# pvphan/camera-calibration

Hardware: AMD Instinct MI355X
Metric: LM iters/sec & residuals/sec, 10k-view checkerboard @1/2/4/8 GPU (higher is better)
Workload: dtype f64

## Files before the change

### camera-calibration_amd/csrc/kernels.hpp

```cpp
#pragma once
#include "point_model.hpp"
#include <stdint.h>
#include <type_traits>

namespace calib {

constexpr int kTile = 256;
constexpr int kGramChunk = 512;
constexpr int kGramUnroll = 4;
constexpr int kGRows = 0;
constexpr int kGStride = 96;
__host__ __device__ __forceinline__ constexpr int gvSlot(int L, int j) { return j < 5 ? L + 1 + j : 16 + L + 2; }
__host__ __device__ __forceinline__ constexpr int gvOfSlot(int L, int slot) {
    const int m = slot >> 4, n = (slot & 15) - L;
    return (m == 0 && n >= 1 && n <= 5) ? n - 1 : ((m == 1 && n == 2) ? 5 : -1);
}
constexpr int kPartStride = 112;
constexpr int kMaxL = 10;

constexpr int kEmitZero = 256;
constexpr int kEmitTile = 264;
constexpr int kEmitTabSize = kGStride + kPartStride;
inline void buildEmitTable(int C, uint32_t* tab ) {
    const int L = C - 6;
// ... 19 lines not shown
        for (int c = 0; c < 16; ++c) tab[kGRows + m * 16 + c] = entry(L + m, c);
    for (int j = 0; j < 6; ++j) tab[gvSlot(L, j)] = gentry(L + j);
    uint32_t* part = tab + kGStride;
    for (int r = 0; r < L; ++r)
        for (int c = 0; c < L; ++c) part[r * L + c] = entry(r, c);
    for (int c = 0; c < L; ++c) part[L * L + c] = gentry(c);
    part[L * L + L] = sse;
}

__host__ __device__ __forceinline__ constexpr int64_t jIndex(int64_t p, int c, int C) {
    return ((p >> 2) * C + c) * 4 + (p & 3);
}
constexpr int kSchurThreads = 256;
constexpr int kMaxSchurBlocks = 1024;

typedef double d4 __attribute__((ext_vector_type(4)));
typedef float f4 __attribute__((ext_vector_type(4)));

__device__ __forceinline__ double2 lane_gather(double2 v, int srcLane) {
    const int a = srcLane << 2;
    int2 lo = __builtin_bit_cast(int2, v.x), hi = __builtin_bit_cast(int2, v.y);
    lo.x = __builtin_amdgcn_ds_bpermute(a, lo.x);  lo.y = __builtin_amdgcn_ds_bpermute(a, lo.y);
    hi.x = __builtin_amdgcn_ds_bpermute(a, hi.x);  hi.y = __builtin_amdgcn_ds_bpermute(a, hi.y);
    double2 o;
    o.x = __builtin_bit_cast(double, lo);  o.y = __builtin_bit_cast(double, hi);
    return o;
}
__device__ __forceinline__ float2 lane_gather(float2 v, int srcLane) {
    const int a = srcLane << 2;
    float2 o;
    o.x = __builtin_bit_cast(float, __builtin_amdgcn_ds_bpermute(a, __builtin_bit_cast(int, v.x)));
    o.y = __builtin_bit_cast(float, __builtin_amdgcn_ds_bpermute(a, __builtin_bit_cast(int, v.y)));
    return o;
}

struct LMState {
    double lam, err_cur, last_err, lam_min, lam_max, err_min;
    int cur;
    int round;
    int iters;
    int max_iters;
    int done;
    int error;
    int accepted_last;
    int fixed_mask;
    int* notify;
    double dc[kMaxL];
    double B[kMaxL * kMaxL];
    double gc[kMaxL];
};

__host__ __device__ constexpr int variantSize(int L) { return 2 * L * L + 2 * L + 2; }
__host__ __device__ constexpr int reduceSize(int L) { return 2 * variantSize(L); }

__device__ __forceinline__ const double* selectP(const double* P0, const double* P1,
                                                 const LMState* st, int sel) {
    if (sel == 0) return P0;
    return (st->cur ^ 1) ? P1 : P0;
}

template <typename T>
__global__ void view_setup_kernel(const double* __restrict__ P0, const double* __restrict__ P1,
                                  const LMState* __restrict__ st, int sel, int L,
                                  const int* __restrict__ view_ext, int nv, T* __restrict__ VC) {
    if (sel && st->done) return;
    const int j = blockIdx.x * blockDim.x + threadIdx.x;
// ... 160 lines not shown
        gacc += __shfl_xor(gacc, 16, 64);
        gacc += __shfl_xor(gacc, 32, 64);
        eacc += __shfl_xor(eacc, 16, 64);
        eacc += __shfl_xor(eacc, 32, 64);
    }
    double* Gbase = sel ? ((st->cur ^ 1) ? G1 : G0) : G0;
#pragma unroll
    for (int reg = 0; reg < 4; ++reg) stile[wave][(k + 4 * reg) * 16 + c] = acc[reg];
    if (k == 0) stile[wave][256 + c] = gacc;
    if (lane == 0) stile[wave][272] = eacc;
    __syncthreads();
    if (threadIdx.x < L * L + L + 1) {
        const int t = threadIdx.x;
        const int idx = t < L * L ? (t / L) * 16 + t % L : (t < L * L + L ? 256 + (t - L * L) : 272);
        part[(int64_t)(part_base + blockIdx.x) * kPartStride + t] =
            (stile[0][idx] + stile[1][idx]) + (stile[2][idx] + stile[3][idx]);
    }
    if (sub == 0 && valid) {
        double* G = Gbase + (int64_t)item * kGStride;
        for (int i = lane; i < kGStride; i += 64) {
            const int j = gvOfSlot(L, i);
            const int idx = j >= 0 ? 256 + L + j : (L + i / 16) * 16 + i % 16;
            double t = stile[wave][idx];
            for (int w = 1; w < wpi; ++w) t += stile[wave + w][idx];
            G[i] = t;
        }
    }
}

constexpr int kFusedRowChunks = 17;
constexpr int kFusedRows = 32;
constexpr int kFusedWaves = 4;

template <typename T, int C>
struct FusedSlab {
    using T2 = typename Pair<T>::type;
    static constexpr bool MF32 = sizeof(T) == 4;
    static constexpr int RS = kFusedRowChunks, ROWS = kFusedRows, WAVES = kFusedWaves;
    static constexpr bool RCOL = C < 16;
    static constexpr bool ONES = !RCOL;
    static constexpr int SIZE = MF32 ? ROWS * RS : ROWS * 16 + ROWS / 2;
    static constexpr int BYTES = WAVES * SIZE * (int)sizeof(T2);
    static_assert(SIZE * sizeof(T2) >= 2 * kEmitTile * 8, "tiles must fit the wave's slab");
    static __device__ __forceinline__ constexpr int rowOff(int r) { return MF32 ? r * RS : r * 16 + (r >> 1); }
    static __device__ __forceinline__ int pointOf(int lane) {
        return MF32 ? lane : ((lane & 48) | ((lane & 7) << 1) | ((lane >> 3) & 1));
    }
    static __device__ __forceinline__ void initRows(T2* slab, int lane) {
        if (lane < ROWS) {
            T2 c3, c4;
            c3.x = T(1); c3.y = ONES ? T(1) : T(0);
            c4.x = T(0); c4.y = T(1);
            slab[rowOff(lane) + 3] = c3;
            if (!ONES) slab[rowOff(lane) + 4] = c4;
            T* zr = reinterpret_cast<T*>(slab + rowOff(lane));
            zr[1] = T(0); zr[2] = T(0); zr[5] = T(0);
        }
    }
    static __device__ __forceinline__ double* tileU(T2* slab) { return reinterpret_cast<double*>(slab); }
    static __device__ __forceinline__ double* tileV(T2* slab) { return tileU(slab) + kEmitTile; }
    static __device__ __forceinline__ void writePartial(const unsigned char* smem, const uint32_t* emit_tab, double* part) {
        if ((int)threadIdx.x < kPartStride) {
            const uint32_t t = emit_tab[kGStride + threadIdx.x];
            const double* T0 = reinterpret_cast<const double*>(smem);
            double o = 0.0;
#pragma unroll
            for (int w = 0; w < WAVES; ++w) {
                const double* TUw = reinterpret_cast<const double*>(reinterpret_cast<const T2*>(T0) + w * SIZE);
                o += TUw[t & 0xffff] + (TUw + kEmitTile)[t >> 16];
            }
            part[(int64_t)blockIdx.x * kPartStride + threadIdx.x] = o;
        }
    }
};

struct BlockAcc {
    double d0u = 0.0, d0v = 0.0, d1u = 0.0, d1v = 0.0, d2u = 0.0;
    int bi, bj, trow, tcol0, tcol1, tcol2;
    __device__ __forceinline__ explicit BlockAcc(int lane) {
        const int k = lane >> 4;
        bi = (lane >> 2) & 3; bj = lane & 3;
        trow = 4 * bi + k; tcol0 = 4 * bi + bj; tcol1 = 4 * ((bi + 1) & 3) + bj; tcol2 = 4 * ((bi + 2) & 3) + bj;
    }
    __device__ __forceinline__ void contract(const double2& ja, const double2& jb, double ha, double hc) {
        d0u = __builtin_amdgcn_mfma_f64_4x4x4f64(ja.x, ja.x, d0u, 0, 0, 0);
        d0v = __builtin_amdgcn_mfma_f64_4x4x4f64(ja.y, ja.y, d0v, 0, 0, 0);
        d1u = __builtin_amdgcn_mfma_f64_4x4x4f64(ja.x, jb.x, d1u, 0, 0, 0);
        d1v = __builtin_amdgcn_mfma_f64_4x4x4f64(ja.y, jb.y, d1v, 0, 0, 0);
        d2u = __builtin_amdgcn_mfma_f64_4x4x4f64(ha, hc, d2u, 0, 0, 0);
    }
    __device__ __forceinline__ void park(double* TU, double* TV) const {
        TU[trow * 16 + tcol0] = d0u;  TV[trow * 16 + tcol0] = d0v;
        TU[trow * 16 + tcol1] = d1u;  TV[trow * 16 + tcol1] = d1v;
        TU[tcol1 * 16 + trow] = d1u;  TV[tcol1 * 16 + trow] = d1v;
        double* T2nd = bi < 2 ? TU : TV;
        T2nd[trow * 16 + tcol2] = d2u;
        T2nd[tcol2 * 16 + trow] = d2u;
    }
};

template <int MODEL, typename T, bool G44, bool MULTI>
__global__ __launch_bounds__(64 * kFusedWaves, (sizeof(T) == 4 ? (MULTI ? 5 : 6)
                                                             : (ModelTraits<MODEL>::C == 16 ? 4 : 3))) void fused_kernel(const double* __restrict__ P0, const double* __restrict__ P1,
                                                    const typename Pair<T>::type* __restrict__ uv,
                                                    const typename Pair<T>::type* __restrict__ XY,
                                                    const T* __restrict__ Z, const T* __restrict__ VC,
                                                    const int64_t* __restrict__ item_pt0,
                                                    const int* __restrict__ item_n,
                                                    const int* __restrict__ item_view, int n_items,
                                                    int uniform_n, int ipw, int wpi,
                                                    const uint32_t* __restrict__ emit_tab,
                                                    const LMState* __restrict__ st, int sel,
                                                    double* __restrict__ G0, double* __restrict__ G1,
                                                    double* __restrict__ part) {
    using T2 = typename Pair<T>::type;
    constexpr int C = ModelTraits<MODEL>::C;
    using Slab = FusedSlab<T, C>;
    constexpr int RS = Slab::RS, ROWS = Slab::ROWS, WAVES = Slab::WAVES, SLAB = Slab::SIZE;
    constexpr bool MF32 = Slab::MF32, RCOL = Slab::RCOL, ONES = Slab::ONES;
    __shared__ __attribute__((aligned(16))) unsigned char smem[Slab::BYTES];
    if (sel && st->done) return;
    const double* P = selectP(P0, P1, st, sel);
    const int lane = threadIdx.x & 63;
    const int wave = __builtin_amdgcn_readfirstlane(threadIdx.x >> 6);
    const int lw = wpi == 4 ? 2 : (wpi == 2 ? 1 : 0);
    const int sub = wave & (wpi - 1);
    static_assert(!(G44 && MULTI), "multi-item waves exist for the tile forms only");
    const int item_first = MULTI ? (blockIdx.x * WAVES + wave) * ipw : blockIdx.x * (WAVES >> lw) + (wave >> lw);
    const bool valid = item_first < n_items;
    int item = item_first;
    const int c = lane & 15, k = lane >> 4;
    const int sl = MF32 ? lane : ((lane & 48) | ((lane & 7) << 1) | ((lane >> 3) & 1));
    T2* slab = reinterpret_cast<T2*>(smem) + wave * SLAB;
    d4 acc = {0.0, 0.0, 0.0, 0.0}, acc2 = {0.0, 0.0, 0.0, 0.0};
    BlockAcc blk(lane);
    double* Gbase = sel ? ((st->cur ^ 1) ? G1 : G0) : G0;
    auto emitDirect = [&](int it) {
        constexpr int L = C - 6, RESROW = RCOL ? 15 : 4;
        double* G = Gbase + (int64_t)it * kGStride;
#pragma unroll
        for (int reg = 0; reg < 4; ++reg) {
            const int row = MF32 ? 4 * k + reg : k + 4 * reg;
            double val = acc[reg] + acc2[reg];
            if (ONES) {
                const int lo = __builtin_amdgcn_update_dpp(0, __double2loint(acc2[reg]), 0x111, 0xf, 0xf, false);
                const int hi = __builtin_amdgcn_update_dpp(0, __double2hiint(acc2[reg]), 0x111, 0xf, 0xf, false);
                const double fromLeft = __hiloint2double(hi, lo);
                val = c == 3 ? acc[reg] : (c == 4 ? fromLeft : val);
            }
            if (row >= L && row < L + 6) {
                const int slot = kGRows + (row - L) * 16 + c;
                if (gvOfSlot(L, slot) < 0) G[slot] = (RCOL && c == 15) ? 0.0 : val;
            } else if (row == RESROW) {
                if (c >= L && c < L + 6) G[gvSlot(L, c - L)] = val;
            }
        }
    };
    if (valid) {
        int64_t pbeg = uniform_n ? (int64_t)item * uniform_n : item_pt0[item];
        const int n = uniform_n ? uniform_n : item_n[item];
        const int item_last = MULTI ? (item_first + ipw < n_items ? item_first + ipw : n_items) - 1 : item_first;
        const int per = ((((n + 3) >> 2) + wpi - 1) >> lw) << 2;
        const int qbeg = sub * per;
        const int qend = qbeg + per < n ? qbeg + per : n;
        Shared<MODEL, T> sp;
        sp.load(P);
        Slab::initRows(slab, lane);
        int64_t pn = pbeg + (qbeg + sl < qend ? qbeg + sl : qend - 1);
        T2 m_n = uv[pn], xy_n = XY[pn];
        T z_n = Z[pn];
        for (;; ++item) {
        const T* vc = VC + (int64_t)__builtin_amdgcn_readfirstlane(uniform_n ? item : item_view[item]) * kViewStride;
        for (int q0 = qbeg; q0 < qend; q0 += 64) {
            const int q = q0 + sl;
            const T2 m = m_n, xy = xy_n;
            const T z = z_n;
            if (q0 + 64 < qend) {
                pn = pbeg + (q + 64 < qend ? q + 64 : qend - 1);
                m_n = uv[pn]; xy_n = XY[pn]; z_n = Z[pn];
            } else if (MULTI && item < item_last) {
                pn = pbeg + n + (sl < n ? sl : n - 1);
                m_n = uv[pn]; xy_n = XY[pn]; z_n = Z[pn];
            }
            T u, v;
            T2 Jc[C];
            jacobian_point<MODEL, T>(sp, vc, xy.x, xy.y, z, u, v, Jc);
            T2 res;
            res.x = m.x - u;
            res.y = m.y - v;
            constexpr int NCH = C - 5 + 1;
            T2 ch[NCH];
#pragma unroll
            for (int i = 0; i < C - 5; ++i) ch[i] = Jc[5 + i];
            ch[NCH - 1] = res;
            auto colOf = [](int i) { return i < C - 5 ? 5 + i : (RCOL ? 15 : 4); };
#pragma unroll
            for (int i = 0; i + 1 < NCH; i += 2) {
                unsigned a[sizeof(T2) / 4], b[sizeof(T2) / 4];
                __builtin_memcpy(a, &ch[i], sizeof(T2));
                __builtin_memcpy(b, &ch[i + 1], sizeof(T2));
#pragma unroll
                for (int d = 0; d < (int)(sizeof(T2) / 4); ++d) {
                    const auto r = __builtin_amdgcn_permlane32_swap(a[d], b[d], false, false);
// ... 64 lines not shown
                    const T* h2 = reinterpret_cast<const T*>(src + c2) + jh;
                    if (rows >= ROWS) {
#pragma unroll
                        for (int s = 0; s < ROWS / 4; ++s)
                            blk.contract(src[66 * s + c], src[66 * s + c1], h0[2 * 66 * s], h2[2 * 66 * s]);
                    } else {
                        for (int s = 0; s < nfull; ++s)
                            blk.contract(src[66 * s + c], src[66 * s + c1], h0[2 * 66 * s], h2[2 * 66 * s]);
                        if (rows & 3) {
                            const bool live = 4 * nfull + k < rows;
                            T2 ja = src[66 * nfull + c], jb = src[66 * nfull + c1];
                            double ha = h0[2 * 66 * nfull], hc = h2[2 * 66 * nfull];
                            if (!live) { ja.x = T(0); ja.y = T(0); jb.x = T(0); jb.y = T(0); ha = 0.0; hc = 0.0; }
                            blk.contract(ja, jb, ha, hc);
                        }
                    }
                }
            }
        }
        if (!MULTI || item >= item_last) break;
        emitDirect(item);
        {
            constexpr int L = C - 6;
#pragma unroll
            for (int reg = 0; reg < 4; ++reg) {
                const int row = MF32 ? 4 * k + reg : k + 4 * reg;
                const bool ofView = (row >= L && row < L + 6) || (c >= L && c < L + 6);
                acc[reg] = ofView ? 0.0 : acc[reg];
                acc2[reg] = ofView ? 0.0 : acc2[reg];
            }
        }
        pbeg += n;
        }
    }
    double* TU = Slab::tileU(slab);
    double* TV = Slab::tileV(slab);
    if (!G44 && wpi == 1 && valid) emitDirect(item);
    __builtin_amdgcn_wave_barrier();
    if constexpr (!G44) {
#pragma unroll
        for (int reg = 0; reg < 4; ++reg) {
            const int row = MF32 ? 4 * k + reg : k + 4 * reg;
            TU[row * 16 + c] = acc[reg];
            TV[row * 16 + c] = acc2[reg];
        }
    } else {
        blk.park(TU, TV);
    }
    if (lane == 0) { TU[kEmitZero] = 0.0; TV[kEmitZero] = 0.0; }
    __syncthreads();
    Slab::writePartial(smem, emit_tab, part);
    if ((!G44 && wpi == 1) || sub != 0 || !valid) return;
    double* G = Gbase + (int64_t)item * kGStride;
    if (lane < kGStride / 2) {
        const int i0 = 2 * lane;
        const uint2 t = *reinterpret_cast<const uint2*>(emit_tab + i0);
        double2 o;
        o.x = TU[t.x & 0xffff] + TV[t.x >> 16];
        o.y = TU[t.y & 0xffff] + TV[t.y >> 16];
        for (int w = 1; w < wpi; ++w) {
            const double* TUw = reinterpret_cast<const double*>(slab + w * SLAB);
            const double* TVw = TUw + kEmitTile;
            o.x += TUw[t.x & 0xffff] + TVw[t.x >> 16];
            o.y += TUw[t.y & 0xffff] + TVw[t.y >> 16];
        }
        *reinterpret_cast<double2*>(G + i0) = o;
    }
}

constexpr int kStreamOps = 12;
constexpr int kStreamNoOp = 0x7ffffff0;
inline bool buildStreamOps(int C, int32_t* ops ) {
    uint32_t tab[kEmitTabSize];
    buildEmitTable(C, tab);
    for (int i = 0; i < 64 * kStreamOps; ++i) ops[i] = kStreamNoOp;
    struct Src { int lane, acc; };
    const auto laneOf = [](int k, int b, int x) { return k * 16 + b * 4 + x; };
    const auto locate = [&](int idx, bool vtile) -> Src {
        const int r = idx / 16, c = idx % 16, br = r / 4, bc = c / 4;
        if (bc == br) return {laneOf(r % 4, br, c % 4), vtile ? 1 : 0};
        if (bc == ((br + 1) & 3)) return {laneOf(r % 4, br, c % 4), vtile ? 3 : 2};
        if (br == ((bc + 1) & 3)) return {laneOf(c % 4, bc, r % 4), vtile ? 3 : 2};
        const bool own = vtile ? br >= 2 : br < 2;
        return own ? Src{laneOf(r % 4, br, c % 4), 4} : Src{laneOf(c % 4, bc, r % 4), 4};
// ... 14 lines not shown
            else if (su.acc == 4 && sv.acc == 4) put(su.lane, 4, 2, slot);
            else ok = false;
        } else if (iu != kEmitZero) {
            const Src su = locate(iu, false);
            put(su.lane, su.acc == 0 ? 6 : (su.acc == 2 ? 8 : 10), 1, slot);
        } else {
            const Src sv = locate(iv, true);
            put(sv.lane, sv.acc == 1 ? 7 : (sv.acc == 3 ? 9 : 10), 1, slot);
        }
    }
    return ok;
}

constexpr int kStreamMinBlocks = 4;
template <int MODEL>
__global__ __launch_bounds__(64 * kFusedWaves, kStreamMinBlocks) void fused_stream_kernel(const double* __restrict__ P0, const double* __restrict__ P1,
                                                              const double2* __restrict__ uv, const double2* __restrict__ XY,
                                                              const double* __restrict__ Z, const double* __restrict__ VC,
                                                              int n, int nv, int share,
                                                              const uint32_t* __restrict__ emit_tab,
                                                              const int32_t* __restrict__ stream_ops,
                                                              const LMState* __restrict__ st, int sel,
                                                              double* __restrict__ G0, double* __restrict__ G1,
                                                              double* __restrict__ part) {
    using T = double;
    using T2 = double2;
    constexpr int C = ModelTraits<MODEL>::C, L = C - 6;
    using Slab = FusedSlab<T, C>;
    constexpr int ROWS = Slab::ROWS, WAVES = Slab::WAVES, SLAB = Slab::SIZE;
    constexpr bool RCOL = Slab::RCOL, ONES = Slab::ONES;
    __shared__ __attribute__((aligned(16))) unsigned char smem[Slab::BYTES];
    __shared__ __attribute__((aligned(16))) double svc[WAVES][2 * kViewStride];
    __shared__ __attribute__((aligned(16))) int32_t sops[64 * kStreamOps];
    int fin = 0, useP1 = 0;
    auto readState = [&]() {
        if (sel) {
            fin = st->done;
            useP1 = st->cur ^ 1;
        }
    };
    const int lane = threadIdx.x & 63;
    const int wave = __builtin_amdgcn_readfirstlane(threadIdx.x >> 6);
    const int k = lane >> 4;
    const int sl = Slab::pointOf(lane);
    T2* slab = reinterpret_cast<T2*>(smem) + wave * SLAB;
    BlockAcc blk(lane);
    double* Gbase = G0;
    auto ofView = [](int i) { return i >= L && i < L + 6; };
    const bool keep0 = !(ofView(blk.trow) || ofView(blk.tcol0)), keep1 = !(ofView(blk.trow) || ofView(blk.tcol1)),
               keep2 = !(ofView(blk.trow) || ofView(blk.tcol2));
    {
        const int4* src = reinterpret_cast<const int4*>(stream_ops) + 3 * lane;
        int4* dst = reinterpret_cast<int4*>(sops) + 3 * lane;
        dst[0] = src[0]; dst[1] = src[1]; dst[2] = src[2];
    }
    const int partner = blk.bj * 16 + ((blk.bi + 2) & 3) * 4 + k;
    auto emitView = [&](int slot) {
        typedef unsigned int u2v __attribute__((ext_vector_type(2)));
        const unsigned long long gp = reinterpret_cast<unsigned long long>(Gbase + (int64_t)slot * kGStride);
        const unsigned glo = (unsigned)__builtin_amdgcn_readfirstlane((int)(unsigned)gp);
        const unsigned ghi = (unsigned)__builtin_amdgcn_readfirstlane((int)(unsigned)(gp >> 32));
        double* G = reinterpret_cast<double*>(((unsigned long long)ghi << 32) | (unsigned long long)glo);
        const auto rsrc = __builtin_amdgcn_make_buffer_rsrc(G, 0, kGStride * 8, 0x00020000);
        const int4* o4 = reinterpret_cast<const int4*>(sops) + 3 * lane;
        const int4 oa = o4[0], ob = o4[1];
        double &d0u = blk.d0u, &d0v = blk.d0v, &d1u = blk.d1u, &d1v = blk.d1v, &d2u = blk.d2u;
        const double s0 = d0u + d0v, s1 = d1u + d1v;
        const double dp = __hiloint2double(__builtin_amdgcn_ds_bpermute(partner << 2, __double2hiint(d2u)),
                                           __builtin_amdgcn_ds_bpermute(partner << 2, __double2loint(d2u)));
        const double s2 = d2u + dp;
        auto put = [&](int off, double val) {
            __builtin_amdgcn_raw_buffer_store_b64(__builtin_bit_cast(u2v, val), rsrc, off, 0, 0);
        };
        put(oa.x, s0); put(oa.y, s0);
        put(oa.z, s1); put(oa.w, s1);
        put(ob.x, s2); put(ob.y, s2);
        if (ONES) {
            const int4 oc = o4[2];
            put(ob.z, d0u); put(ob.w, d0v);
            put(oc.x, d1u); put(oc.y, d1v);
            put(oc.z, d2u);
        }
        d0u = keep0 ? d0u : 0.0;  d0v = keep0 ? d0v : 0.0;
        d1u = keep1 ? d1u : 0.0;  d1v = keep1 ? d1v : 0.0;
        d2u = keep2 ? d2u : 0.0;
    };
    const int n4 = n >> 2;
    const int w = blockIdx.x * WAVES + wave;
    const long long gt = (long long)nv * n4, g0 = (long long)w * share;
    const bool valid = g0 < gt;
    if (valid) {
        const int p0 = (int)(4 * g0);
        const int p1 = (int)(4 * (g0 + share < gt ? g0 + share : gt));
        int va = __builtin_amdgcn_readfirstlane(p0 / n);
        int vend = (va + 1) * n;
        int slot = p0 != va * n ? nv + w : va;
        Shared<MODEL, T> sp, spB;
        sp.load(P0);
        spB = sp;
        if (sel) spB.load(P1);
        Slab::initRows(slab, lane);
        int pn = p0 + sl < p1 ? p0 + sl : p1 - 1;
        T2 m_n = uv[pn], xy_n = XY[pn];
        T z_n = Z[pn];
        auto straddles = [&](int q0, int ve) { return ve > q0 && ve < (q0 + 64 < p1 ? q0 + 64 : p1); };
        const int vcLast = nv * kViewStride - 1;
        auto stagedLoad = [&](int view) {
            const int i = view * kViewStride + (lane < 2 * kViewStride ? lane : 2 * kViewStride - 1);
            return VC[i < vcLast ? i : vcLast];
        };
        double vc_n = 0.0;
        double vcs[kViewStride];
#pragma unroll
        for (int i = 0; i < kViewStride; ++i) vcs[i] = 0.0;
        auto scalarLoad = [&](int view) {
            const T* s = VC + (int64_t)__builtin_amdgcn_readfirstlane(view) * kViewStride;
#pragma unroll
            for (int i = 0; i < kViewStride - 1; ++i) vcs[i] = s[i];
        };
        bool strad = straddles(p0, vend);
        if (strad) vc_n = stagedLoad(va); else scalarLoad(va);
        readState();
        if (fin) return;
        if (useP1) sp = spB;
        Gbase = useP1 ? G1 : G0;
        const T2* src = slab + Slab::rowOff(k);
        const int c = lane & 15, c1 = (c + 4) & 15, c2 = (c + 8) & 15, jh = (lane >> 3) & 1;
        const T* h0 = reinterpret_cast<const T*>(src + c) + jh;
        const T* h2 = reinterpret_cast<const T*>(src + c2) + jh;
        PointState<MODEL, T> pst;
        for (int q0 = p0; q0 < p1; q0 += 64) {
            const int qe = q0 + 64 < p1 ? q0 + 64 : p1;
            const int q = q0 + sl;
            const T2 m = m_n, xy = xy_n;
            const T z = z_n;
            const double vcx = vc_n;
            const bool more = q0 + 64 < p1;
            const bool passes = vend < qe;
            const int ve2 = passes ? vend + n : vend, va2 = passes ? va + 1 : va;
            const bool strad2 = more && straddles(q0 + 64, ve2);
            const int vfirst2 = ve2 <= q0 + 64 ? va2 + 1 : va2;
            if (more) {
                pn = q + 64 < p1 ? q + 64 : p1 - 1;
                m_n = uv[pn]; xy_n = XY[pn]; z_n = Z[pn];
                if (strad2) vc_n = stagedLoad(va2);
            }
            T u, v;
            T2 Jc[C];
            if (!strad) {
                jacobian_stage_a<MODEL, T>(sp, vcs, xy.x, xy.y, z, pst);
                jacobian_stage_b<MODEL, T>(sp, vcs, pst, u, v, Jc);
            } else {
                double* sv = svc[wave];
                if (lane < 2 * kViewStride) sv[lane] = vcx;
                __builtin_amdgcn_wave_barrier();
                const int qc = q < p1 ? q : p1 - 1;
                const double2* s2 = reinterpret_cast<const double2*>(sv + (qc >= vend ? kViewStride : 0));
                T vcl[kViewStride];
// ... 83 lines not shown
                        runFixed(integral_constant<int, 0>{}, integral_constant<int, JB>{});
                        nextView();
                        runFixed(integral_constant<int, JB>{}, integral_constant<int, NG>{});
                    };
                    switch (jb) {
                    case 0: boundaryAt(integral_constant<int, 0>{}); break;
                    case 1: boundaryAt(integral_constant<int, 1>{}); break;
                    case 2: boundaryAt(integral_constant<int, 2>{}); break;
                    case 3: boundaryAt(integral_constant<int, 3>{}); break;
                    case 4: boundaryAt(integral_constant<int, 4>{}); break;
                    case 5: boundaryAt(integral_constant<int, 5>{}); break;
                    case 6: boundaryAt(integral_constant<int, 6>{}); break;
                    default: boundaryAt(integral_constant<int, 7>{}); break;
                    }
                } else {
                    const int sb = jb < ng ? jb : ng;
                    auto runGroups = [&](int from, int to) {
                        switch (from) {
#define CALIB_GROUP_CASE(S) case S: if (to <= S) break; blk.contract(src[66 * S + c], src[66 * S + c1], h0[2 * 66 * S], h2[2 * 66 * S]); [[fallthrough]];
                        CALIB_GROUP_CASE(0) CALIB_GROUP_CASE(1) CALIB_GROUP_CASE(2) CALIB_GROUP_CASE(3)
                        CALIB_GROUP_CASE(4) CALIB_GROUP_CASE(5) CALIB_GROUP_CASE(6) CALIB_GROUP_CASE(7)
#undef CALIB_GROUP_CASE
                        default: break;
                        }
                    };
                    runGroups(0, sb);
                    if (jb < ng) {
                        nextView();
                        runGroups(sb, ng);
                    }
                }
            }
        }
        emitView(slot);
    } else {
        readState();
        if (fin) return;
    }
    {
        double* TU = Slab::tileU(slab);
        double* TV = Slab::tileV(slab);
        __builtin_amdgcn_wave_barrier();
        blk.park(TU, TV);
        if (lane == 0) { TU[kEmitZero] = 0.0; TV[kEmitZero] = 0.0; }
    }
    __syncthreads();
    Slab::writePartial(smem, emit_tab, part);
}

struct StreamMap { int share, n4, nv; };
__host__ __device__ __forceinline__ int stream_extra_item(const StreamMap& sm, int v) {
    if (sm.share == 0) return -1;
    const unsigned first = (unsigned)v * (unsigned)sm.n4, last = first + (unsigned)sm.n4 - 1u;
    const unsigned w = last / (unsigned)sm.share;
    return w * (unsigned)sm.share > first ? sm.nv + (int)w : -1;
}

struct ViewSpan { int i0, nitems, extra; };
template <bool STREAM>
__device__ __forceinline__ ViewSpan view_span(const int* __restrict__ view_item0, const StreamMap& sm, int v) {
    ViewSpan s;
    s.i0 = view_item0 ? view_item0[v] : v;
    s.nitems = view_item0 ? view_item0[v + 1] - s.i0 : 1;
    s.extra = STREAM ? stream_extra_item(sm, v) : -1;
    return s;
}

__device__ __forceinline__ constexpr int tri(int m, int n) { return m * (m + 1) / 2 + n; }

__device__ __forceinline__ double rsqrt_nr(double d) {
    const double r = __builtin_amdgcn_rsq(d);
    const double e = __builtin_fma(-(d * r), r, 1.0);
    const double p = __builtin_fma(0.375, e, 0.5);
    return __builtin_fma(r * e, p, r);
}

template <int N>
__device__ __forceinline__ double row_bcast(double v) {
    return __hiloint2double(__builtin_amdgcn_update_dpp(0, __double2hiint(v), 0x150 + N, 0xf, 0xf, false),
                            __builtin_amdgcn_update_dpp(0, __double2loint(v), 0x150 + N, 0xf, 0xf, false));
// ... 161 lines not shown
    __shared__ double sfail[kSchurViewsPerBlock];
    __shared__ double stile[kSchurBlock / 64][256];
    const int tid = threadIdx.x, lane = tid & 63, wave = tid >> 6, c = tid & 15, grp = tid >> 4, k = lane >> 4;

    if (blockIdx.y == 2) {
        constexpr int NF = L * L + L + 1;
        double* out = part + (int64_t)blockIdx.x * VA;
        const int t = tid & 127, half = tid >> 7;
        double s0 = 0.0, s1 = 0.0, s2 = 0.0, s3 = 0.0;
        if (t < NF) {
            const int64_t step = (int64_t)gridDim.x * 2;
            int64_t it = (int64_t)blockIdx.x * 2 + half;
            const double* src = bpart + t;
            for (; it + 3 * step < n_bpart; it += 4 * step) {
                s0 += src[it * kPartStride];
                s1 += src[(it + step) * kPartStride];
                s2 += src[(it + 2 * step) * kPartStride];
                s3 += src[(it + 3 * step) * kPartStride];
            }
            for (; it < n_bpart; it += step) s0 += src[it * kPartStride];
        }
        if (st->done) return;
        double* sh = &stile[0][0];
        sh[tid] = (s0 + s1) + (s2 + s3);
        __syncthreads();
        if (tid < NF) {
            const double tot = sh[tid] + sh[128 + tid];
            out[tid < L * L ? tid : (tid < L * L + L ? 2 * L * L + (tid - L * L) : kSse)] = tot;
        }
        return;
    }

    const double* G = blockIdx.y ? G1 : G0;
    double V[21], b[6];
    int v0 = blockIdx.x * kSchurViewsPerBlock;
    if (v0 + grp < nv) load_view_head<L, WIDE>(G, view_span<STREAM>(view_item0, sm, v0 + grp), c, V, b);
    if (st->done) return;
    const bool boot = st->round == 0;
    const int cand = st->cur ^ 1;
    const int variant = (int)blockIdx.y == cand ? 0 : 1;
    double* out = part + ((int64_t)variant * gridDim.x + blockIdx.x) * VA;
    if (variant == 1 && boot) {
        for (int i = tid; i < VA; i += kSchurBlock) out[i] = 0.0;
        return;
    }
    const double lam = variant == 0 ? (boot ? st->lam : st->lam / 10) : st->lam * 10;

    d4 acc = {0.0, 0.0, 0.0, 0.0};
    double nfail = 0.0;
    const int stride = gridDim.x * kSchurViewsPerBlock;
    while (v0 < nv) {
        double z[6];
#pragma unroll
        for (int m = 0; m < 6; ++m) z[m] = 0.0;
        const bool live = v0 + grp < nv;
        const bool more = v0 + stride + grp < nv;
        double rn[6];
        if (WIDE && more)
            request_head_rows(G, view_span<STREAM>(view_item0, sm, v0 + stride + grp), c, rn);
        if (live) {
            double invd[6];
            const bool ok = eliminate(V, b, lam, invd, z);
            if (c > L) {
#pragma unroll
                for (int m = 0; m < 6; ++m) z[m] = 0.0;
            }
            if (!ok) nfail += 1.0;
        }
        v0 += stride;
        if (more) {
            if constexpr (WIDE) {
                expand_head_rows<L>(rn, c, V, b);
            } else {
                load_view_head<L, false>(G, view_span<STREAM>(view_item0, sm, v0 + grp), c, V, b);
            }
        }
#pragma unroll
        for (int m = 0; m < 6; ++m) acc = __builtin_amdgcn_mfma_f64_16x16x4f64(z[m], z[m], acc, 0, 0, 0);
    }
// ... 68 lines not shown
        u32x4 mine;
        mine.x = (unsigned)__double2loint(t); mine.y = x.epoch;
        mine.z = (unsigned)__double2hiint(t); mine.w = x.epoch;
        if (lane != x.rank) cell_store(dst, mine);
        const unsigned long long* src = own + 2 * ((int64_t)(lane * 2 + par) * kPeerStride + i);
        const long long t0 = wall_clock64();
        v = t;
        while (lane != x.rank) {
            const u32x4 c = cell_load(src);
            if (c.y == x.epoch && c.w == x.epoch) {
                v = __hiloint2double((int)c.z, (int)c.x);
                break;
            }
            if ((unsigned long long)(wall_clock64() - t0) > x.timeout_ticks) {
                __hip_atomic_store(x.fault, 1, __ATOMIC_RELAXED, __HIP_MEMORY_SCOPE_AGENT);
                if (x.notify) __hip_atomic_store(x.notify, 2, __ATOMIC_RELAXED, __HIP_MEMORY_SCOPE_SYSTEM);
                v = __builtin_nan("");
                break;
            }
            __builtin_amdgcn_s_sleep(2);
        }
    }
    double acc = 0.0;
    for (int r = 0; r < x.world; ++r) acc += __shfl(v, r, 64);
    return acc;
}

__global__ __launch_bounds__(64) void reduce_kernel(const double* __restrict__ part, int nblocks, int VA,
                                                    const LMState* __restrict__ st,
                                                    double* __restrict__ red, PeerExchange x) {
    const int i = blockIdx.x, lane = threadIdx.x;
    const int variant = i / VA, idx = i - variant * VA;
    const double* src = part + (int64_t)variant * nblocks * VA + idx;
    double v[kMaxSchurBlocks / 64];
#pragma unroll
    for (int j = 0; j < kMaxSchurBlocks / 64; ++j) {
        const int b = lane + 64 * j;
        v[j] = b < nblocks ? src[(int64_t)b * VA] : 0.0;
    }
#pragma unroll
    for (int w = 1; w < kMaxSchurBlocks / 64; w *= 2)
#pragma unroll
        for (int j = 0; j + w < kMaxSchurBlocks / 64; j += 2 * w) v[j] += v[j + w];
    double t = v[0];
#pragma unroll
    for (int off = 32; off > 0; off >>= 1) t += __shfl_down(t, off, 64);
    const bool done = st->done != 0;
    if (x.world > 1) t = peer_sum(x, i, __shfl(t, 0, 64), lane);
    if (done) return;
    if (lane == 0) red[i] = t;
}

__global__ __launch_bounds__(64) void peer_selftest_kernel(PeerExchange x, int round, int* __restrict__ mismatches) {
    const int i = blockIdx.x, lane = threadIdx.x;
    const double mine = (double)(x.rank + 1) * (i + 1) + round;
    const double got = peer_sum(x, i, mine, lane);
    const double want = 0.5 * x.world * (x.world + 1.0) * (i + 1) + (double)round * x.world;
    if (lane == 0 && !(got == want)) atomicAdd(mismatches, 1);
}

__global__ __launch_bounds__(256) void sse_reduce_kernel(const double* __restrict__ sse_part, int64_t n,
                                                         double* __restrict__ out) {
    __shared__ double ssum[256];
    const int tid = threadIdx.x;
    double e = 0.0;
    for (int64_t i = tid; i < n; i += 256) e += sse_part[i];
    ssum[tid] = e;
    __syncthreads();
    for (int s = 128; s > 0; s >>= 1) {
        if (tid < s) ssum[tid] += ssum[tid + s];
        __syncthreads();
    }
    if (tid == 0) out[0] = ssum[0];
}

constexpr int kDppXor1 = 0xB1;
constexpr int kDppXor2 = 0x4E;
constexpr int kDppHalfMirror = 0x141;
constexpr int kDppMirror = 0x140;

// ... 36 lines not shown
        take(dpp_d<kDppXor1>(best), dpp_i<kDppXor1>(bi));
        take(dpp_d<kDppXor2>(best), dpp_i<kDppXor2>(bi));
        take(dpp_d<kDppHalfMirror>(best), dpp_i<kDppHalfMirror>(bi));
        take(dpp_d<kDppMirror>(best), dpp_i<kDppMirror>(bi));
        if (!(best > 0.0)) singular = true;
        double prow[N + 1];
        if (WAVE0) {
            const int sb = __builtin_amdgcn_readfirstlane(bi);
#pragma unroll
            for (int j = col; j <= N; ++j)
                prow[j] = __hiloint2double(__builtin_amdgcn_readlane(__double2hiint(row[j]), sb),
                                           __builtin_amdgcn_readlane(__double2loint(row[j]), sb));
        } else {
#pragma unroll
            for (int j = col; j <= N; ++j) prow[j] = __shfl(row[j], bi, 16);
        }
        if (i == bi) {
            used = true;
            myCol = col;
        } else {
            const double f = div_nr(row[col], prow[col]);
#pragma unroll
            for (int j = col + 1; j <= N; ++j) row[j] -= f * prow[j];
            row[col] = 0.0;
        }
    }
    double piv = 1.0;
#pragma unroll
    for (int j = 0; j < N; ++j) if (myCol == j) piv = row[j];
    d = row[N] / piv;
    return singular;
}

__device__ __forceinline__ double readlane_d(double v, int lane) {
    return __hiloint2double(__builtin_amdgcn_readlane(__double2hiint(v), lane),
                            __builtin_amdgcn_readlane(__double2loint(v), lane));
}

template <int N>
__device__ __forceinline__ bool spd_solve_wave0(double (&row)[N + 1], int i, double (&x)[N]) {
    bool ok = true;
    double rinv[N];
#pragma unroll
    for (int j = 0; j < N; ++j) {
        double p[N + 1];
#pragma unroll
        for (int k = j; k <= N; ++k) p[k] = readlane_d(row[k], j);
        if (!(p[j] > 0.0)) ok = false;
        rinv[j] = div_nr(1.0, p[j]);
        if (i > j) {
            const double f = row[j] * rinv[j];
#pragma unroll
            for (int k = j + 1; k <= N; ++k) row[k] -= f * p[k];
        }
    }
    double acc = row[N];
#pragma unroll
    for (int j = N - 1; j >= 0; --j) {
        const double xj = readlane_d(acc, j) * rinv[j];
        x[j] = xj;
        if (i < j) acc -= row[j] * xj;
    }
    return ok;
}

struct LMDecision { int cur; double lam; bool acc; };
__device__ __forceinline__ LMDecision lm_decide(int cur, double lam, int round, double err_cand, double err_cur) {
    if (round == 0) return {cur ^ 1, lam, false};
    if (err_cand < err_cur) return {cur ^ 1, lam / 10, true};
    return {cur, lam * 10, false};
}

template <int L>
__device__ __forceinline__ bool lm_update_step(const LMState* __restrict__ in, LMState* __restrict__ out,
                                               const double* __restrict__ red, double* __restrict__ P0,
                                               double* __restrict__ P1, double* __restrict__ trace,
                                               bool writer, int i, int& cur_out, double& lam_out,
                                               double (&dc)[L]) {
    constexpr int VA = variantSize(L);
    constexpr int kNfail = 2 * L * L + 2 * L, kSse = kNfail + 1;
    const bool w0 = writer && i == 0;
    double* Pb[2] = {P0, P1};
    int cur = in->cur;
    const int round = in->round;
    const double err_cand = red[kSse];
    double lam = in->lam;
    double sA[L], sB[L], bA[L], bS[L];
    double rhsA = 0.0, rhsB = 0.0, gA = 0.0, gS = 0.0;
#pragma unroll
    for (int j = 0; j < L; ++j) { sA[j] = 0.0; sB[j] = 0.0; bA[j] = 0.0; bS[j] = 0.0; }
    if (i < L) {
#pragma unroll
        for (int j = 0; j < L; ++j) {
            sA[j] = red[L * L + i * L + j];
            sB[j] = red[VA + L * L + i * L + j];
            bA[j] = red[i * L + j];
            bS[j] = in->B[i * L + j];
        }
        rhsA = red[2 * L * L + L + i];
        rhsB = red[VA + 2 * L * L + L + i];
        gA = red[2 * L * L + i];
        gS = in->gc[i];
    }
    const double nfailA = red[kNfail], nfailB = red[VA + kNfail];
    if (in->done) {
        if (writer) for (int j = i; j < (int)(sizeof(LMState) / 8); j += 16)
            reinterpret_cast<double*>(out)[j] = reinterpret_cast<const double*>(in)[j];
        return false;
    }
    bool useB = false;
    bool done = false;
    double err_cur_new = err_cand, last_err = err_cand;
    int iters = in->iters, accepted = 0;
    const double err_cur = in->err_cur;
    const LMDecision dec = lm_decide(cur, lam, round, err_cand, err_cur);
    if (round > 0) {
        const int it = round - 1;
        if (trace && writer) {
            double* row = trace + (int64_t)it * (5 + L);
            if (i < L) row[5 + i] = Pb[cur][i];
            if (i == 0) { row[0] = it; row[1] = err_cur; row[2] = err_cand; row[3] = lam; row[4] = dec.acc ? 1.0 : 0.0; }
        }
        useB = !dec.acc;
        done = !(in->lam_min < dec.lam && dec.lam < in->lam_max) || err_cur < in->err_min || it + 1 >= in->max_iters;
        last_err = err_cur;
        err_cur_new = dec.acc ? err_cand : err_cur;
        iters = it + 1;
        accepted = dec.acc ? 1 : 0;
    }
    cur = dec.cur;
    lam = dec.lam;
    int error = 0;
    if (!done && (useB ? nfailB : nfailA) > 0.0) { error = -3; done = true; }

    double row[L + 1], brow[L];
    const double gci = useB ? gS : gA;
#pragma unroll
    for (int j = 0; j < L; ++j) {
        brow[j] = useB ? bS[j] : bA[j];
        row[j] = brow[j] - (useB ? sB[j] : sA[j]);
    }
    row[L] = gci - (useB ? rhsB : rhsA);
#pragma unroll
    for (int j = 0; j < L; ++j) if (j == i) row[j] += lam * brow[j];
    const int fixed_mask = in->fixed_mask;
    const bool fixed_i = (fixed_mask >> i) & 1;
    if (fixed_mask != 0) {
#pragma unroll
        for (int j = 0; j < L; ++j) {
            const bool fixed_j = (fixed_mask >> j) & 1;
            row[j] = (fixed_i || fixed_j) ? (j == i ? 1.0 : 0.0) : row[j];
        }
        row[L] = fixed_i ? 0.0 : row[L];
    }
    if (!done) {
        double saved[L + 1];
#pragma unroll
        for (int j = 0; j <= L; ++j) saved[j] = row[j];
        if (!spd_solve_wave0<L>(row, i, dc)) {
            int myCol = -1;
            double d = 0.0;
            if (gauss_jordan16<L, true>(saved, i, myCol, d)) { error = -3; done = true; }
#pragma unroll
            for (int c = 0; c < L; ++c) dc[c] = group_sum16(myCol == c ? d : 0.0);
        }
    } else {
#pragma unroll
        for (int c = 0; c < L; ++c) dc[c] = 0.0;
    }

    if (writer) {
        if (i < L) {
#pragma unroll
            for (int j = 0; j < L; ++j) out->B[i * L + j] = brow[j];
            out->gc[i] = gci;
            double dci = 0.0;
#pragma unroll
            for (int c = 0; c < L; ++c) if (c == i) dci = dc[c];
            out->dc[i] = dci;
            if (!done) Pb[cur ^ 1][i] = fixed_i ? Pb[cur][i] : Pb[cur][i] + dci;
        }
        if (w0) {
            out->lam = lam; out->err_cur = err_cur_new; out->last_err = last_err;
            out->lam_min = in->lam_min; out->lam_max = in->lam_max; out->err_min = in->err_min;
            out->cur = cur; out->round = round + 1; out->iters = iters; out->max_iters = in->max_iters;
            out->done = done ? 1 : 0; out->error = error; out->accepted_last = accepted; out->fixed_mask = fixed_mask;
            out->notify = in->notify;
            if (done && in->notify) __hip_atomic_store(in->notify, 1, __ATOMIC_RELAXED, __HIP_MEMORY_SCOPE_SYSTEM);
        }
    }
    cur_out = cur;
    lam_out = lam;
    return !done;
}

template <int L, typename T>
__device__ __forceinline__ void finish_view(const double (&V)[21], const double (&invd)[6], const double (&z)[6],
                                            double coef, int c, int v, const int* __restrict__ view_ext,
                                            const double* __restrict__ Pc, double* __restrict__ Pn,
                                            T* __restrict__ VC) {
    double w[6];
#pragma unroll
    for (int m = 0; m < 6; ++m) w[m] = group_sum16(coef * z[m]);
    double d[6];
    backward6(V, invd, w, d);
    const int64_t o = L + 6 * (int64_t)view_ext[v];
    double en[6];
#pragma unroll
    for (int m = 0; m < 6; ++m) en[m] = Pc[o + m] + d[m];
    if (c < 6) {
        double ev = en[0];
#pragma unroll
        for (int m = 1; m < 6; ++m) ev = (c == m) ? en[m] : ev;
        Pn[o + c] = ev;
    }
    const double deg = 0.017453292519943295;
    double sn[3], cs[3];
    {
        const int a = c & 3;
        const double th = (a == 1 ? en[1] : (a == 2 ? en[2] : en[0])) * deg;
        double s1, c1;
// ... 801 lines not shown
```

Before: 30.76 billion.

## Issue LM state and parameter loads early to overlap scalar memory latency

Reorders the loads of the LM state word, the parameter vectors and the emit-table entries so they are issued before the first point-data loads and consumed later. In the f64 path, both parameter sets are loaded across lanes in one shot and broadcast with readlane instead of being loaded twice. Empty asm constraints pin the values in scalar registers and sched_barrier holds the order. The goal is to hide the load latency at kernel start and in the Schur and solve kernels, at the cost of more live registers and more fragile scheduling.

New measurement: 31.42 billion (median of 6 runs). 2.2% higher.

```diff
diff --git a/camera-calibration_amd/csrc/kernels.hpp b/camera-calibration_amd/csrc/kernels.hpp
--- a/camera-calibration_amd/csrc/kernels.hpp
+++ b/camera-calibration_amd/csrc/kernels.hpp
@@ -75,6 +75,11 @@
     o.x = __builtin_bit_cast(float, __builtin_amdgcn_ds_bpermute(a, __builtin_bit_cast(int, v.x)));
     o.y = __builtin_bit_cast(float, __builtin_amdgcn_ds_bpermute(a, __builtin_bit_cast(int, v.y)));
     return o;
+}
+
+__device__ __forceinline__ double readlane_d(double v, int lane) {
+    return __hiloint2double(__builtin_amdgcn_readlane(__double2hiint(v), lane),
+                            __builtin_amdgcn_readlane(__double2loint(v), lane));
 }
 
 struct LMState {
@@ -301,6 +306,31 @@
 constexpr int kFusedRows = 32;
 constexpr int kFusedWaves = 4;
 
+struct StateWords {
+    int fin = 0, useP1 = 0;
+    __device__ __forceinline__ void request(const LMState* __restrict__ st, int sel) {
+        if (sel) { fin = st->done; useP1 = st->cur; }
+    }
+    __device__ __forceinline__ void take(int sel) {
+        asm("" : "+s"(fin), "+s"(useP1));
+        useP1 = sel ? useP1 ^ 1 : 0;
+    }
+};
+template <int L>
+__device__ __forceinline__ double request_shared_both(const double* __restrict__ P0, const double* __restrict__ P1,
+                                                      int sel, int lane) {
+    const int pl = lane & 15;
+    return (((lane & 16) && sel) ? P1 : P0)[pl < L ? pl : L - 1];
+}
+template <int MODEL, typename T>
+__device__ __forceinline__ void shared_from_lanes(Shared<MODEL, T>& sp, double pboth, int useP1) {
+    constexpr int L = ModelTraits<MODEL>::C - 6;
+    double pv[L];
+#pragma unroll
+    for (int j = 0; j < L; ++j) pv[j] = readlane_d(pboth, (useP1 ? 16 : 0) + j);
+    sp.load(pv);
+}
+
 template <typename T, int C>
 struct FusedSlab {
     using T2 = typename Pair<T>::type;
@@ -328,9 +358,15 @@
     }
     static __device__ __forceinline__ double* tileU(T2* slab) { return reinterpret_cast<double*>(slab); }
     static __device__ __forceinline__ double* tileV(T2* slab) { return tileU(slab) + kEmitTile; }
-    static __device__ __forceinline__ void writePartial(const unsigned char* smem, const uint32_t* emit_tab, double* part) {
+    static __device__ __forceinline__ uint32_t partEntry(const uint32_t* __restrict__ emit_tab) {
+        uint32_t t = 0;
+        int i = kGStride + (int)threadIdx.x;
+        asm("" : "+v"(i));
+        if ((int)threadIdx.x < kPartStride) t = emit_tab[i];
+        return t;
+    }
+    static __device__ __forceinline__ void writePartial(const unsigned char* smem, uint32_t t, double* part) {
         if ((int)threadIdx.x < kPartStride) {
-            const uint32_t t = emit_tab[kGStride + threadIdx.x];
             const double* T0 = reinterpret_cast<const double*>(smem);
             double o = 0.0;
 #pragma unroll
@@ -388,8 +424,12 @@
     constexpr int RS = Slab::RS, ROWS = Slab::ROWS, WAVES = Slab::WAVES, SLAB = Slab::SIZE;
     constexpr bool MF32 = Slab::MF32, RCOL = Slab::RCOL, ONES = Slab::ONES;
     __shared__ __attribute__((aligned(16))) unsigned char smem[Slab::BYTES];
-    if (sel && st->done) return;
-    const double* P = selectP(P0, P1, st, sel);
+    StateWords sw;
+    if constexpr (MF32) {
+        sw.request(st, sel);
+        sw.take(sel);
+        if (sw.fin) return;
+    }
     const int lane = threadIdx.x & 63;
     const int wave = __builtin_amdgcn_readfirstlane(threadIdx.x >> 6);
     const int lw = wpi == 4 ? 2 : (wpi == 2 ? 1 : 0);
@@ -403,7 +443,7 @@
     T2* slab = reinterpret_cast<T2*>(smem) + wave * SLAB;
     d4 acc = {0.0, 0.0, 0.0, 0.0}, acc2 = {0.0, 0.0, 0.0, 0.0};
     BlockAcc blk(lane);
-    double* Gbase = sel ? ((st->cur ^ 1) ? G1 : G0) : G0;
+    double* Gbase = (MF32 && sw.useP1) ? G1 : G0;
     auto emitDirect = [&](int it) {
         constexpr int L = C - 6, RESROW = RCOL ? 15 : 4;
         double* G = Gbase + (int64_t)it * kGStride;
@@ -433,11 +473,25 @@
         const int qbeg = sub * per;
         const int qend = qbeg + per < n ? qbeg + per : n;
         Shared<MODEL, T> sp;
-        sp.load(P);
-        Slab::initRows(slab, lane);
+        double pboth = 0.0;
+        if constexpr (MF32) {
+            sp.load(sw.useP1 ? P1 : P0);
+            Slab::initRows(slab, lane);
+        } else {
+            pboth = request_shared_both<C - 6>(P0, P1, sel, lane);
+        }
         int64_t pn = pbeg + (qbeg + sl < qend ? qbeg + sl : qend - 1);
         T2 m_n = uv[pn], xy_n = XY[pn];
         T z_n = Z[pn];
+        if constexpr (!MF32) {
+            sw.request(st, sel);
+            __builtin_amdgcn_sched_barrier(0);
+            sw.take(sel);
+            Slab::initRows(slab, lane);
+            if (sw.fin) return;
+            shared_from_lanes<MODEL, T>(sp, pboth, sw.useP1);
+            Gbase = sw.useP1 ? G1 : G0;
+        }
         for (;; ++item) {
         const T* vc = VC + (int64_t)__builtin_amdgcn_readfirstlane(uniform_n ? item : item_view[item]) * kViewStride;
         for (int q0 = qbeg; q0 < qend; q0 += 64) {
@@ -568,9 +622,15 @@
         }
         pbeg += n;
         }
+    } else if constexpr (!MF32) {
+        sw.request(st, sel);
+        sw.take(sel);
+        if (sw.fin) return;
+        Gbase = sw.useP1 ? G1 : G0;
     }
     double* TU = Slab::tileU(slab);
     double* TV = Slab::tileV(slab);
+    const uint32_t tpart = Slab::partEntry(emit_tab);
     if (!G44 && wpi == 1 && valid) emitDirect(item);
     __builtin_amdgcn_wave_barrier();
     if constexpr (!G44) {
@@ -585,7 +645,7 @@
     }
     if (lane == 0) { TU[kEmitZero] = 0.0; TV[kEmitZero] = 0.0; }
     __syncthreads();
-    Slab::writePartial(smem, emit_tab, part);
+    Slab::writePartial(smem, tpart, part);
     if ((!G44 && wpi == 1) || sub != 0 || !valid) return;
     double* G = Gbase + (int64_t)item * kGStride;
     if (lane < kGStride / 2) {
@@ -666,13 +726,8 @@
     __shared__ __attribute__((aligned(16))) unsigned char smem[Slab::BYTES];
     __shared__ __attribute__((aligned(16))) double svc[WAVES][2 * kViewStride];
     __shared__ __attribute__((aligned(16))) int32_t sops[64 * kStreamOps];
-    int fin = 0, useP1 = 0;
-    auto readState = [&]() {
-        if (sel) {
-            fin = st->done;
-            useP1 = st->cur ^ 1;
-        }
-    };
+    asm("" : "+s"(share) : "s"(P0), "s"(P1), "s"(uv), "s"(XY), "s"(Z), "s"(stream_ops), "s"(n), "s"(nv), "s"(sel));
+    StateWords sw;
     const int lane = threadIdx.x & 63;
     const int wave = __builtin_amdgcn_readfirstlane(threadIdx.x >> 6);
     const int k = lane >> 4;
@@ -683,11 +738,6 @@
     auto ofView = [](int i) { return i >= L && i < L + 6; };
     const bool keep0 = !(ofView(blk.trow) || ofView(blk.tcol0)), keep1 = !(ofView(blk.trow) || ofView(blk.tcol1)),
                keep2 = !(ofView(blk.trow) || ofView(blk.tcol2));
-    {
-        const int4* src = reinterpret_cast<const int4*>(stream_ops) + 3 * lane;
-        int4* dst = reinterpret_cast<int4*>(sops) + 3 * lane;
-        dst[0] = src[0]; dst[1] = src[1]; dst[2] = src[2];
-    }
     const int partner = blk.bj * 16 + ((blk.bi + 2) & 3) * 4 + k;
     auto emitView = [&](int slot) {
         typedef unsigned int u2v __attribute__((ext_vector_type(2)));
@@ -723,17 +773,16 @@
     const int w = blockIdx.x * WAVES + wave;
     const long long gt = (long long)nv * n4, g0 = (long long)w * share;
     const bool valid = g0 < gt;
+    uint32_t tpart = 0;
     if (valid) {
         const int p0 = (int)(4 * g0);
         const int p1 = (int)(4 * (g0 + share < gt ? g0 + share : gt));
         int va = __builtin_amdgcn_readfirstlane(p0 / n);
         int vend = (va + 1) * n;
         int slot = p0 != va * n ? nv + w : va;
-        Shared<MODEL, T> sp, spB;
-        sp.load(P0);
-        spB = sp;
-        if (sel) spB.load(P1);
-        Slab::initRows(slab, lane);
+        const int4* opsrc = reinterpret_cast<const int4*>(stream_ops) + 3 * lane;
+        const int4 op0 = opsrc[0], op1 = opsrc[1], op2 = opsrc[2];
+        const double pboth = request_shared_both<L>(P0, P1, sel, lane);
         int pn = p0 + sl < p1 ? p0 + sl : p1 - 1;
         T2 m_n = uv[pn], xy_n = XY[pn];
         T z_n = Z[pn];
@@ -754,10 +803,18 @@
         };
         bool strad = straddles(p0, vend);
         if (strad) vc_n = stagedLoad(va); else scalarLoad(va);
-        readState();
-        if (fin) return;
-        if (useP1) sp = spB;
-        Gbase = useP1 ? G1 : G0;
+        sw.request(st, sel);
+        __builtin_amdgcn_sched_barrier(0);
+        sw.take(sel);
+        {
+            int4* dst = reinterpret_cast<int4*>(sops) + 3 * lane;
+            dst[0] = op0; dst[1] = op1; dst[2] = op2;
+        }
+        Slab::initRows(slab, lane);
+        if (sw.fin) return;
+        Shared<MODEL, T> sp;
+        shared_from_lanes<MODEL, T>(sp, pboth, sw.useP1);
+        Gbase = sw.useP1 ? G1 : G0;
         const T2* src = slab + Slab::rowOff(k);
         const int c = lane & 15, c1 = (c + 4) & 15, c2 = (c + 8) & 15, jh = (lane >> 3) & 1;
         const T* h0 = reinterpret_cast<const T*>(src + c) + jh;
@@ -907,10 +964,13 @@
                 }
             }
         }
+        tpart = Slab::partEntry(emit_tab);
         emitView(slot);
     } else {
-        readState();
-        if (fin) return;
+        sw.request(st, sel);
+        tpart = emit_tab[kGStride + ((int)threadIdx.x < kPartStride ? (int)threadIdx.x : 0)];
+        sw.take(sel);
+        if (sw.fin) return;
     }
     {
         double* TU = Slab::tileU(slab);
@@ -920,7 +980,7 @@
         if (lane == 0) { TU[kEmitZero] = 0.0; TV[kEmitZero] = 0.0; }
     }
     __syncthreads();
-    Slab::writePartial(smem, emit_tab, part);
+    Slab::writePartial(smem, tpart, part);
 }
 
 struct StreamMap { int share, n4, nv; };
@@ -1148,19 +1208,22 @@
     }
 
     const double* G = blockIdx.y ? G1 : G0;
+    int st_done = st->done, st_cur = st->cur, st_round = st->round;
+    double st_lam = st->lam;
     double V[21], b[6];
     int v0 = blockIdx.x * kSchurViewsPerBlock;
     if (v0 + grp < nv) load_view_head<L, WIDE>(G, view_span<STREAM>(view_item0, sm, v0 + grp), c, V, b);
-    if (st->done) return;
-    const bool boot = st->round == 0;
-    const int cand = st->cur ^ 1;
+    asm("" : "+s"(st_done), "+s"(st_cur), "+s"(st_round), "+s"(st_lam));
+    if (st_done) return;
+    const bool boot = st_round == 0;
+    const int cand = st_cur ^ 1;
     const int variant = (int)blockIdx.y == cand ? 0 : 1;
     double* out = part + ((int64_t)variant * gridDim.x + blockIdx.x) * VA;
     if (variant == 1 && boot) {
         for (int i = tid; i < VA; i += kSchurBlock) out[i] = 0.0;
         return;
     }
-    const double lam = variant == 0 ? (boot ? st->lam : st->lam / 10) : st->lam * 10;
+    const double lam = variant == 0 ? (boot ? st_lam : st_lam / 10) : st_lam * 10;
 
     d4 acc = {0.0, 0.0, 0.0, 0.0};
     double nfail = 0.0;
@@ -1295,6 +1358,7 @@
     const int i = blockIdx.x, lane = threadIdx.x;
     const int variant = i / VA, idx = i - variant * VA;
     const double* src = part + (int64_t)variant * nblocks * VA + idx;
+    int st_done = st->done;
     double v[kMaxSchurBlocks / 64];
 #pragma unroll
     for (int j = 0; j < kMaxSchurBlocks / 64; ++j) {
@@ -1308,7 +1372,8 @@
     double t = v[0];
 #pragma unroll
     for (int off = 32; off > 0; off >>= 1) t += __shfl_down(t, off, 64);
-    const bool done = st->done != 0;
+    asm("" : "+s"(st_done));
+    const bool done = st_done != 0;
     if (x.world > 1) t = peer_sum(x, i, __shfl(t, 0, 64), lane);
     if (done) return;
     if (lane == 0) red[i] = t;
@@ -1411,10 +1476,6 @@
     return singular;
 }
 
-__device__ __forceinline__ double readlane_d(double v, int lane) {
-    return __hiloint2double(__builtin_amdgcn_readlane(__double2hiint(v), lane),
-                            __builtin_amdgcn_readlane(__double2loint(v), lane));
-}
 
 template <int N>
 __device__ __forceinline__ bool spd_solve_wave0(double (&row)[N + 1], int i, double (&x)[N]) {
@@ -1481,8 +1542,12 @@
         gA = red[2 * L * L + i];
         gS = in->gc[i];
     }
-    const double nfailA = red[kNfail], nfailB = red[VA + kNfail];
-    if (in->done) {
+    double nfailA = red[kNfail], nfailB = red[VA + kNfail];
+    int in_done = in->done, in_iters = in->iters, in_max_iters = in->max_iters, in_fixed_mask = in->fixed_mask;
+    double in_err_cur = in->err_cur, in_lam_min = in->lam_min, in_lam_max = in->lam_max, in_err_min = in->err_min;
+    asm("" : "+s"(in_done), "+s"(in_iters), "+s"(in_max_iters), "+s"(in_fixed_mask), "+s"(in_err_cur), "+s"(in_lam_min),
+             "+s"(in_lam_max), "+s"(in_err_min), "+s"(nfailA), "+s"(nfailB));
+    if (in_done) {
         if (writer) for (int j = i; j < (int)(sizeof(LMState) / 8); j += 16)
             reinterpret_cast<double*>(out)[j] = reinterpret_cast<const double*>(in)[j];
         return false;
@@ -1490,8 +1555,8 @@
     bool useB = false;
     bool done = false;
     double err_cur_new = err_cand, last_err = err_cand;
-    int iters = in->iters, accepted = 0;
-    const double err_cur = in->err_cur;
+    int iters = in_iters, accepted = 0;
+    const double err_cur = in_err_cur;
     const LMDecision dec = lm_decide(cur, lam, round, err_cand, err_cur);
     if (round > 0) {
         const int it = round - 1;
@@ -1501,7 +1566,7 @@
             if (i == 0) { row[0] = it; row[1] = err_cur; row[2] = err_cand; row[3] = lam; row[4] = dec.acc ? 1.0 : 0.0; }
         }
         useB = !dec.acc;
-        done = !(in->lam_min < dec.lam && dec.lam < in->lam_max) || err_cur < in->err_min || it + 1 >= in->max_iters;
+        done = !(in_lam_min < dec.lam && dec.lam < in_lam_max) || err_cur < in_err_min || it + 1 >= in_max_iters;
         last_err = err_cur;
         err_cur_new = dec.acc ? err_cand : err_cur;
         iters = it + 1;
@@ -1522,7 +1587,7 @@
     row[L] = gci - (useB ? rhsB : rhsA);
 #pragma unroll
     for (int j = 0; j < L; ++j) if (j == i) row[j] += lam * brow[j];
-    const int fixed_mask = in->fixed_mask;
+    const int fixed_mask = in_fixed_mask;
     const bool fixed_i = (fixed_mask >> i) & 1;
     if (fixed_mask != 0) {
 #pragma unroll
@@ -1561,11 +1626,14 @@
         }
         if (w0) {
             out->lam = lam; out->err_cur = err_cur_new; out->last_err = last_err;
-            out->lam_min = in->lam_min; out->lam_max = in->lam_max; out->err_min = in->err_min;
-            out->cur = cur; out->round = round + 1; out->iters = iters; out->max_iters = in->max_iters;
+            const LMState* pass = in;
+            asm("" : "+s"(pass));
+            out->lam_min = pass->lam_min; out->lam_max = pass->lam_max; out->err_min = pass->err_min;
+            out->cur = cur; out->round = round + 1; out->iters = iters; out->max_iters = pass->max_iters;
             out->done = done ? 1 : 0; out->error = error; out->accepted_last = accepted; out->fixed_mask = fixed_mask;
-            out->notify = in->notify;
-            if (done && in->notify) __hip_atomic_store(in->notify, 1, __ATOMIC_RELAXED, __HIP_MEMORY_SCOPE_SYSTEM);
+            int* const notify = pass->notify;
+            out->notify = notify;
+            if (done && notify) __hip_atomic_store(notify, 1, __ATOMIC_RELAXED, __HIP_MEMORY_SCOPE_SYSTEM);
         }
     }
     cur_out = cur;
```
